# CPJKU/beat_this

Measured on NVIDIA H100. Metric: clips/sec (30 s audio->beats, final0), higher is better.
Workload: dtype f16

## Files before the change

### beat_this_b200/csrc/kernels_fused.cu

```cuda
#include <cstdio>
#include <cstdlib>
#include <cstring>

#include "tc_common.cuh"

namespace bt {

constexpr int FU_WARPS = 8;
constexpr int FU_THREADS = 32 * FU_WARPS;

__device__ __forceinline__ void stage_weight(h16* dst, const h16* __restrict__ src, int rows, int cols) {
  const int vpr = cols / 8;
  for (int i = threadIdx.x; i < rows * vpr; i += blockDim.x) {
    const int r = i / vpr, v = i - r * vpr;
    *reinterpret_cast<uint4*>(dst + r * (cols + 8) + v * 8) = __ldg(reinterpret_cast<const uint4*>(src + static_cast<int64_t>(r) * cols) + v);
  }
}
__device__ __forceinline__ uint32_t lds32(const h16* p) { return *reinterpret_cast<const uint32_t*>(p); }
template <int LD>
__device__ __forceinline__ void b_frag(const h16* sW, int nb, int ks, int lane, uint32_t& b0, uint32_t& b1) {
  const h16* p = sW + (nb * 8 + (lane >> 2)) * LD + ks * 16 + 2 * (lane & 3);
  b0 = lds32(p);
  b1 = lds32(p + 8);
}

template <int C>
__global__ void __launch_bounds__(FU_THREADS, C == 32 ? 4 : 2)
fused_qkv_kernel(const h16* __restrict__ wqkv, const float* __restrict__ X, const float* __restrict__ wg,
                 const float* __restrict__ bg, const float* __restrict__ rope_cos, const float* __restrict__ rope_sin,
                 h16* __restrict__ qkv, float* __restrict__ gates, int64_t M, int L, int F, int posmode, float qscale) {
  constexpr int LD = C + 8, KS = C / 16, NB = 3 * C / 8, heads = C / 32;
  extern __shared__ uint4 fu_smem[];
  h16* sW = reinterpret_cast<h16*>(fu_smem);
  stage_weight(sW, wqkv, 3 * C, C);
  __syncthreads();
  const int warp = threadIdx.x >> 5, lane = threadIdx.x & 31, q = lane & 3;
  const int64_t ngroups = (M + 15) / 16;
  for (int64_t g = static_cast<int64_t>(blockIdx.x) * FU_WARPS + warp; g < ngroups; g += static_cast<int64_t>(gridDim.x) * FU_WARPS) {
    int64_t m[2];
    bool ok[2];
    float xs[2][C / 4];
#pragma unroll
    for (int r = 0; r < 2; ++r) {
      m[r] = g * 16 + (lane >> 2) + 8 * r;
      ok[r] = m[r] < M;
#pragma unroll
      for (int j = 0; j < C / 4; j += 2) {
        const float2 v = ok[r] ? *reinterpret_cast<const float2*>(X + m[r] * C + 16 * (j >> 2) + 8 * ((j >> 1) & 1) + 2 * q)
                               : make_float2(0.f, 0.f);
        xs[r][j] = v.x;
        xs[r][j + 1] = v.y;
      }
    }
#pragma unroll
    for (int r = 0; r < 2; ++r) {
      float ss = 0.f;
#pragma unroll
      for (int j = 0; j < C / 4; ++j) ss = fmaf(xs[r][j], xs[r][j], ss);
      ss += __shfl_xor_sync(0xffffffffu, ss, 1);
      ss += __shfl_xor_sync(0xffffffffu, ss, 2);
      const float inv = 1.0f / fmaxf(sqrtf(ss), 1e-12f);
#pragma unroll
      for (int j = 0; j < C / 4; ++j) xs[r][j] *= inv;
    }
#pragma unroll
    for (int h = 0; h < heads; ++h) {
#pragma unroll
      for (int r = 0; r < 2; ++r) {
        float a = 0.f;
#pragma unroll
        for (int j = 0; j < C / 4; j += 2) {
          const float2 w = __ldg(reinterpret_cast<const float2*>(wg + h * C + 16 * (j >> 2) + 8 * ((j >> 1) & 1) + 2 * q));
          a = fmaf(xs[r][j], w.x, fmaf(xs[r][j + 1], w.y, a));
        }
        a += __shfl_xor_sync(0xffffffffu, a, 1);
        a += __shfl_xor_sync(0xffffffffu, a, 2);
        if (q == 0 && ok[r]) gates[m[r] * heads + h] = sigmoidf_(a + __ldg(bg + h));
      }
    }
    uint32_t a[KS][4];
#pragma unroll
    for (int ks = 0; ks < KS; ++ks) {
      a[ks][0] = pack_h16x2(xs[0][4 * ks], xs[0][4 * ks + 1]);
      a[ks][1] = pack_h16x2(xs[1][4 * ks], xs[1][4 * ks + 1]);
      a[ks][2] = pack_h16x2(xs[0][4 * ks + 2], xs[0][4 * ks + 3]);
      a[ks][3] = pack_h16x2(xs[1][4 * ks + 2], xs[1][4 * ks + 3]);
    }
    const float* cs[2];
    const float* sn[2];
#pragma unroll
    for (int r = 0; r < 2; ++r) {
      const int pos = ok[r] ? (posmode == 0 ? static_cast<int>(m[r] % L) : static_cast<int>((m[r] / L) % F)) : 0;
      cs[r] = rope_cos + pos * 16;
      sn[r] = rope_sin + pos * 16;
    }
#pragma unroll
    for (int nb = 0; nb < NB; ++nb) {
      float acc[4] = {0.f, 0.f, 0.f, 0.f};
#pragma unroll
      for (int ks = 0; ks < KS; ++ks) {
        uint32_t b0, b1;
        b_frag<LD>(sW, nb, ks, lane, b0, b1);
        mma_16816(acc, a[ks], b0, b1);
      }
      const int n = nb * 8 + 2 * q;
      const int which = (nb * 8) / C;
#pragma unroll
      for (int r = 0; r < 2; ++r) {
        float v0 = acc[2 * r], v1 = acc[2 * r + 1];
        if (which < 2) {
          const float sc = which == 0 ? qscale : 1.0f;
          const int i = ((n - which * C) & 31) >> 1;
          const float co = __ldg(cs[r] + i), si = __ldg(sn[r] + i);
          const float x0 = v0, x1 = v1;
          v0 = (x0 * co - x1 * si) * sc;
          v1 = (x1 * co + x0 * si) * sc;
        }
        if (ok[r]) *reinterpret_cast<uint32_t*>(qkv + m[r] * (3 * C) + n) = pack_h16x2(v0, v1);
      }
    }
  }
}

template <int C, bool OP>
__global__ void __launch_bounds__(FU_THREADS, C == 32 ? 3 : 2)
fused_ff_kernel(const h16* __restrict__ w1, const h16* __restrict__ w2, const h16* __restrict__ wo,
                const h16* __restrict__ O, float* __restrict__ X, const float* __restrict__ b1,
                const float* __restrict__ b2, h16* __restrict__ xb_out, int64_t M) {
  constexpr int HID = 4 * C, LD1 = C + 8, LD2 = HID + 8, KS = C / 16, NB = C / 8, HS = HID / 16;
  extern __shared__ uint4 fu_smem[];
  h16* sW1 = reinterpret_cast<h16*>(fu_smem);
  h16* sW2 = sW1 + HID * LD1;
  h16* sWo = sW2 + C * LD2;
  stage_weight(sW1, w1, HID, C);
  stage_weight(sW2, w2, C, HID);
  if constexpr (OP) stage_weight(sWo, wo, C, C);
  __syncthreads();
  const int warp = threadIdx.x >> 5, lane = threadIdx.x & 31, q = lane & 3;
  const int64_t ngroups = (M + 15) / 16;
  for (int64_t g = static_cast<int64_t>(blockIdx.x) * FU_WARPS + warp; g < ngroups; g += static_cast<int64_t>(gridDim.x) * FU_WARPS) {
    int64_t m[2];
    bool ok[2];
#pragma unroll
    for (int r = 0; r < 2; ++r) {
      m[r] = g * 16 + (lane >> 2) + 8 * r;
      ok[r] = m[r] < M;
    }
    float acc[NB][4];
#pragma unroll
    for (int nb = 0; nb < NB; ++nb)
#pragma unroll
      for (int r = 0; r < 2; ++r) {
        const float2 v = ok[r] ? *reinterpret_cast<const float2*>(X + m[r] * C + nb * 8 + 2 * q) : make_float2(0.f, 0.f);
        acc[nb][2 * r] = v.x;
        acc[nb][2 * r + 1] = v.y;
      }
    if constexpr (OP) {
      uint32_t ao[KS][4];
#pragma unroll
      for (int ks = 0; ks < KS; ++ks)
#pragma unroll
        for (int i = 0; i < 4; ++i) {
          const int r = i & 1;
          ao[ks][i] = ok[r] ? *reinterpret_cast<const uint32_t*>(O + m[r] * C + ks * 16 + 8 * (i >> 1) + 2 * q) : 0u;
        }
#pragma unroll
      for (int nb = 0; nb < NB; ++nb)
#pragma unroll
        for (int ks = 0; ks < KS; ++ks) {
          uint32_t b0, b1;
          b_frag<LD1>(sWo, nb, ks, lane, b0, b1);
          mma_16816(acc[nb], ao[ks], b0, b1);
        }
    }
    float inv[2];
#pragma unroll
    for (int r = 0; r < 2; ++r) {
      float ss = 0.f;
#pragma unroll
      for (int nb = 0; nb < NB; ++nb) ss = fmaf(acc[nb][2 * r], acc[nb][2 * r], fmaf(acc[nb][2 * r + 1], acc[nb][2 * r + 1], ss));
      ss += __shfl_xor_sync(0xffffffffu, ss, 1);
      ss += __shfl_xor_sync(0xffffffffu, ss, 2);
      inv[r] = 1.0f / fmaxf(sqrtf(ss), 1e-12f);
    }
    uint32_t a[KS][4];
#pragma unroll
    for (int ks = 0; ks < KS; ++ks) {
      a[ks][0] = pack_h16x2(acc[2 * ks][0] * inv[0], acc[2 * ks][1] * inv[0]);
      a[ks][1] = pack_h16x2(acc[2 * ks][2] * inv[1], acc[2 * ks][3] * inv[1]);
      a[ks][2] = pack_h16x2(acc[2 * ks + 1][0] * inv[0], acc[2 * ks + 1][1] * inv[0]);
      a[ks][3] = pack_h16x2(acc[2 * ks + 1][2] * inv[1], acc[2 * ks + 1][3] * inv[1]);
    }
#pragma unroll
    for (int nb = 0; nb < NB; ++nb) {
      const float2 b = __ldg(reinterpret_cast<const float2*>(b2 + nb * 8 + 2 * q));
      acc[nb][0] += b.x; acc[nb][1] += b.y;
      acc[nb][2] += b.x; acc[nb][3] += b.y;
    }
#pragma unroll 2
    for (int j = 0; j < HS; ++j) {
      float hh[2][4];
#pragma unroll
      for (int t = 0; t < 2; ++t) {
        hh[t][0] = hh[t][1] = hh[t][2] = hh[t][3] = 0.f;
#pragma unroll
        for (int ks = 0; ks < KS; ++ks) {
          uint32_t b0, b1;
          b_frag<LD1>(sW1, 2 * j + t, ks, lane, b0, b1);
          mma_16816(hh[t], a[ks], b0, b1);
        }
        const float2 b = __ldg(reinterpret_cast<const float2*>(b1 + (2 * j + t) * 8 + 2 * q));
        hh[t][0] = gelu_tanh_fast(hh[t][0] + b.x); hh[t][1] = gelu_tanh_fast(hh[t][1] + b.y);
        hh[t][2] = gelu_tanh_fast(hh[t][2] + b.x); hh[t][3] = gelu_tanh_fast(hh[t][3] + b.y);
      }
      const uint32_t ah[4] = {pack_h16x2(hh[0][0], hh[0][1]), pack_h16x2(hh[0][2], hh[0][3]), pack_h16x2(hh[1][0], hh[1][1]),
                              pack_h16x2(hh[1][2], hh[1][3])};
#pragma unroll
      for (int nb = 0; nb < NB; ++nb) {
        uint32_t b0, b1;
        b_frag<LD2>(sW2, nb, j, lane, b0, b1);
        mma_16816(acc[nb], ah, b0, b1);
      }
    }
#pragma unroll
    for (int nb = 0; nb < NB; ++nb)
#pragma unroll
      for (int r = 0; r < 2; ++r) {
        if (!ok[r]) continue;
        const int64_t o = m[r] * C + nb * 8 + 2 * q;
        *reinterpret_cast<float2*>(X + o) = make_float2(acc[nb][2 * r], acc[nb][2 * r + 1]);
        if (xb_out) *reinterpret_cast<uint32_t*>(xb_out + o) = pack_h16x2(acc[nb][2 * r], acc[nb][2 * r + 1]);
      }
  }
}

template <int C> constexpr int ff_smem(bool op) { return (4 * C * (C + 8) + C * (4 * C + 8) + (op ? C * (C + 8) : 0)) * 2; }
template <int C> constexpr int qkv_smem() { return 3 * C * (C + 8) * 2; }
template <int C> constexpr int ff_ctas() { return C == 32 ? 3 : 2; }
template <int C> constexpr int qkv_ctas() { return C == 32 ? 4 : 2; }

struct TcFfPlan {
  const void *w1, *w2, *o, *wo;
  int C;
  int64_t M;
  bool outproj;
};

TcFfPlan* tc_ff_plan_create(const void* w1_h16, const void* w2_h16, int C, int64_t M, const void* o_h16,
                            const void* wout_h16, char* err, int errlen) {
  if (C != 32 && C != 64) { snprintf(err, errlen, "fused ff: C must be 32 or 64"); return nullptr; }
  TcFfPlan* p = new TcFfPlan();
  p->w1 = w1_h16; p->w2 = w2_h16; p->o = o_h16; p->wo = wout_h16;
  p->C = C; p->M = M; p->outproj = o_h16 != nullptr && wout_h16 != nullptr;
  return p;
}
void tc_ff_plan_destroy(TcFfPlan* p) { delete p; }

static unsigned fused_grid(int64_t M, int ctas_per_sm) {
  const int64_t ctas = ((M + 15) / 16 + FU_WARPS - 1) / FU_WARPS;
  const int64_t slots = static_cast<int64_t>(g_num_sms) * ctas_per_sm;
  return static_cast<unsigned>(ctas < slots ? ctas : slots);
}

void launch_fused_ff(const TcFfPlan* p, float* X, const float* b1, const float* b2, void* xb_out, cudaStream_t st) {
  const h16* w1 = static_cast<const h16*>(p->w1);
  const h16* w2 = static_cast<const h16*>(p->w2);
  const h16* wo = static_cast<const h16*>(p->wo);
  const h16* o = static_cast<const h16*>(p->o);
  h16* xb = static_cast<h16*>(xb_out);
#define BT_FF_L(CC, OPP)                                                                                            \
  fused_ff_kernel<CC, OPP><<<fused_grid(p->M, ff_ctas<CC>()), FU_THREADS, ff_smem<CC>(OPP), st>>>(w1, w2, wo, o, X, b1, \
                                                                                                  b2, xb, p->M)
  if (p->C == 32) { if (p->outproj) BT_FF_L(32, true); else BT_FF_L(32, false); }
  else { if (p->outproj) BT_FF_L(64, true); else BT_FF_L(64, false); }
#undef BT_FF_L
}

struct TcQkvPlan {
  const void* w;
  int C;
  int64_t M;
};
TcQkvPlan* tc_qkv_plan_create(const void* wqkv_h16, int C, int64_t M, char* err, int errlen) {
  if (C != 32 && C != 64) { snprintf(err, errlen, "fused qkv: C must be 32 or 64"); return nullptr; }
  TcQkvPlan* p = new TcQkvPlan();
  p->w = wqkv_h16; p->C = C; p->M = M;
  return p;
}
void tc_qkv_plan_destroy(TcQkvPlan* p) { delete p; }
void launch_fused_qkv(const TcQkvPlan* p, const float* X, const float* wg, const float* bg, const float* rope_cos,
                      const float* rope_sin, void* qkv, float* gates, int L, int F, int posmode, float qscale,
                      cudaStream_t st) {
  const h16* w = static_cast<const h16*>(p->w);
  h16* out = static_cast<h16*>(qkv);
  if (p->C == 32)
    fused_qkv_kernel<32><<<fused_grid(p->M, qkv_ctas<32>()), FU_THREADS, qkv_smem<32>(), st>>>(w, X, wg, bg, rope_cos, rope_sin, out,
                                                                                             gates, p->M, L, F, posmode, qscale);
  else
    fused_qkv_kernel<64><<<fused_grid(p->M, qkv_ctas<64>()), FU_THREADS, qkv_smem<64>(), st>>>(w, X, wg, bg, rope_cos, rope_sin, out,
                                                                                             gates, p->M, L, F, posmode, qscale);
}

int tc_init_fused(char* err, int errlen) {
  cudaError_t r = cudaFuncSetAttribute(fused_ff_kernel<32, false>, cudaFuncAttributeMaxDynamicSharedMemorySize, ff_smem<32>(false));
  if (r == cudaSuccess) r = cudaFuncSetAttribute(fused_ff_kernel<64, false>, cudaFuncAttributeMaxDynamicSharedMemorySize, ff_smem<64>(false));
  if (r == cudaSuccess) r = cudaFuncSetAttribute(fused_ff_kernel<32, true>, cudaFuncAttributeMaxDynamicSharedMemorySize, ff_smem<32>(true));
  if (r == cudaSuccess) r = cudaFuncSetAttribute(fused_ff_kernel<64, true>, cudaFuncAttributeMaxDynamicSharedMemorySize, ff_smem<64>(true));
  if (r == cudaSuccess) r = cudaFuncSetAttribute(fused_qkv_kernel<32>, cudaFuncAttributeMaxDynamicSharedMemorySize, qkv_smem<32>());
  if (r == cudaSuccess) r = cudaFuncSetAttribute(fused_qkv_kernel<64>, cudaFuncAttributeMaxDynamicSharedMemorySize, qkv_smem<64>());
  if (r != cudaSuccess) {
    snprintf(err, errlen, "cudaFuncSetAttribute(fused_ff_kernel / fused_qkv_kernel) failed: %s", cudaGetErrorString(r));
    return -1;
  }
  return 0;
}

}
```

### beat_this_b200/csrc/kernels_misc.cu

```cuda
#include <cuda_fp16.h>
#include <cstdio>
#include <cstdlib>

#include "bt_kernels.h"
#include "common.cuh"
#include "tc_common.cuh"

namespace bt {

__global__ void __launch_bounds__(128)
stem_kernel(const float* __restrict__ spect, const ChunkSrc* __restrict__ chunks, int L,
            const float* __restrict__ bn1_scale, const float* __restrict__ bn1_shift,
            const float* __restrict__ w, const float* __restrict__ bias, float* __restrict__ out) {
  __shared__ float ws[32 * 12];
  __shared__ float bs[32];
  for (int i = threadIdx.x; i < 32 * 12; i += 128) ws[i] = w[i];
  if (threadIdx.x < 32) bs[threadIdx.x] = bias[threadIdx.x];
  __syncthreads();
  const int t = blockIdx.x * 128 + threadIdx.x;
  const int f = blockIdx.y;
  const int b = blockIdx.z;
  if (t >= L) return;
  const ChunkSrc cs = chunks[b];
  float in[4][3];
#pragma unroll
  for (int dt = 0; dt < 3; ++dt) {
    const int tl = t + dt - 1;
    const bool conv_ok = tl >= 0 && tl < cs.len;
    const int64_t fr = static_cast<int64_t>(cs.start) + tl;
    const bool clip_ok = fr >= 0 && fr < cs.T;
    float4 v = make_float4(0.f, 0.f, 0.f, 0.f);
    if (conv_ok && clip_ok)
      v = *reinterpret_cast<const float4*>(spect + (cs.frame_base + fr) * 128 + 4 * f);
    const float vv[4] = {v.x, v.y, v.z, v.w};
#pragma unroll
    for (int df = 0; df < 4; ++df)
      in[df][dt] = conv_ok ? fmaf(vv[df], bn1_scale[4 * f + df], bn1_shift[4 * f + df]) : 0.f;
  }
  float* op = out + ((static_cast<int64_t>(b) * 32 + f) * L + t) * 32;
#pragma unroll
  for (int c4 = 0; c4 < 8; ++c4) {
    float r[4];
#pragma unroll
    for (int i = 0; i < 4; ++i) {
      const int co = c4 * 4 + i;
      float a = bs[co];
#pragma unroll
      for (int df = 0; df < 4; ++df)
#pragma unroll
        for (int dt = 0; dt < 3; ++dt) a = fmaf(in[df][dt], ws[co * 12 + df * 3 + dt], a);
      r[i] = gelu_fast(a);
    }
    reinterpret_cast<float4*>(op)[c4] = make_float4(r[0], r[1], r[2], r[3]);
  }
}

__global__ void __launch_bounds__(256)
zero_tail_kernel(uint4* __restrict__ buf, const ChunkSrc* __restrict__ chunks, int F, int L, int row_vec) {
  const int plane = blockIdx.x;
  const int len = chunks[plane / F].len;
  const int64_t n = static_cast<int64_t>(L - len) * row_vec;
  uint4* p = buf + (static_cast<int64_t>(plane) * L + len) * row_vec;
  for (int64_t i = threadIdx.x; i < n; i += 256) p[i] = make_uint4(0u, 0u, 0u, 0u);
}
void launch_zero_tail(void* buf, int elem_bytes, const ChunkSrc* chunks, int nchunks, int F, int L, int C, cudaStream_t st) {
  zero_tail_kernel<<<nchunks * F, 256, 0, st>>>(reinterpret_cast<uint4*>(buf), chunks, F, L, C * elem_bytes / 16);
}

void launch_stem(const float* spect, const ChunkSrc* chunks, int nchunks, int L, const float* bn1_scale,
                 const float* bn1_shift, const float* w, const float* bias, float* out,
                 cudaStream_t st) {
  dim3 grid(ceil_div(L, 128), 32, nchunks);
  stem_kernel<<<grid, 128, 0, st>>>(spect, chunks, L, bn1_scale, bn1_shift, w, bias, out);
}

template <typename TAct, int C>
__global__ void __launch_bounds__(256)
norm_kernel(const float* __restrict__ x, TAct* __restrict__ xn, int64_t M, float* __restrict__ gates,
            const float* __restrict__ wg, const float* __restrict__ bg, int heads) {
  constexpr int LPR = C / 4 < 32 ? C / 4 : 32;
  constexpr int RPW = 32 / LPR;
  constexpr int VPL = C / 4 / LPR;
  const int lane = threadIdx.x & 31;
  const int64_t warp = static_cast<int64_t>(blockIdx.x) * 8 + (threadIdx.x >> 5);
  const int64_t row = warp * RPW + lane / LPR;
  const int li = lane % LPR;
  const bool ok = row < M;
  const float4* xr = reinterpret_cast<const float4*>(x + (ok ? row : 0) * C);
  float4 v[VPL];
  float ss = 0.f;
#pragma unroll
  for (int i = 0; i < VPL; ++i) {
    v[i] = xr[li + LPR * i];
    ss = fmaf(v[i].x, v[i].x, ss); ss = fmaf(v[i].y, v[i].y, ss);
    ss = fmaf(v[i].z, v[i].z, ss); ss = fmaf(v[i].w, v[i].w, ss);
  }
#pragma unroll
  for (int o = LPR / 2; o > 0; o >>= 1) ss += __shfl_xor_sync(0xffffffffu, ss, o);
  const float inv = 1.0f / fmaxf(sqrtf(ss), 1e-12f);
#pragma unroll
  for (int i = 0; i < VPL; ++i) { v[i].x *= inv; v[i].y *= inv; v[i].z *= inv; v[i].w *= inv; }
  if (gates) {
    for (int h = 0; h < heads; ++h) {
      const float4* w4 = reinterpret_cast<const float4*>(wg + h * C);
      float a = 0.f;
#pragma unroll
      for (int i = 0; i < VPL; ++i) {
        const float4 w = __ldg(w4 + li + LPR * i);
        a = fmaf(v[i].x, w.x, a); a = fmaf(v[i].y, w.y, a); a = fmaf(v[i].z, w.z, a); a = fmaf(v[i].w, w.w, a);
      }
#pragma unroll
      for (int o = LPR / 2; o > 0; o >>= 1) a += __shfl_xor_sync(0xffffffffu, a, o);
      if (ok && li == 0) gates[row * heads + h] = sigmoidf_(a + __ldg(bg + h));
    }
  }
  if (!ok) return;
#pragma unroll
  for (int i = 0; i < VPL; ++i) {
    TAct* dst = xn + row * C + 4 * (li + LPR * i);
    if constexpr (sizeof(TAct) == 4) {
      *reinterpret_cast<float4*>(dst) = v[i];
    } else {
      uint2 u;
      u.x = pack_h16x2(v[i].x, v[i].y);
      u.y = pack_h16x2(v[i].z, v[i].w);
      *reinterpret_cast<uint2*>(dst) = u;
    }
  }
}

template <typename TAct>
static void norm_dispatch(const float* x, void* xn, int64_t M, int C, float* gates, const float* wg, const float* bg,
                          int heads, cudaStream_t st) {
  TAct* o = reinterpret_cast<TAct*>(xn);
#define BT_NORM_CASE(c)                                                                                   \
  case c: {                                                                                               \
    constexpr int rpw = (c / 4 < 32) ? 32 / (c / 4) : 1;                                                  \
    norm_kernel<TAct, c><<<static_cast<unsigned>(ceil_div64(M, 8 * rpw)), 256, 0, st>>>(x, o, M, gates, wg, \
                                                                                          bg, heads);     \
  } break;
  switch (C) {
    BT_NORM_CASE(32) BT_NORM_CASE(64) BT_NORM_CASE(128) BT_NORM_CASE(256) BT_NORM_CASE(512) BT_NORM_CASE(1024)
    default: break;
  }
#undef BT_NORM_CASE
}

void launch_norm(const float* x, void* xn, int64_t M, int C, int act_h16, cudaStream_t st, float* gates,
                 const float* wg, const float* bg, int heads) {
  if (act_h16) norm_dispatch<h16>(x, xn, M, C, gates, wg, bg, heads, st);
  else norm_dispatch<float>(x, xn, M, C, gates, wg, bg, heads, st);
}

__device__ __forceinline__ void load_row32(const float* p, float (&v)[32]) {
#pragma unroll
  for (int i = 0; i < 8; ++i) {
    const float4 q = reinterpret_cast<const float4*>(p)[i];
    v[4 * i] = q.x; v[4 * i + 1] = q.y; v[4 * i + 2] = q.z; v[4 * i + 3] = q.w;
  }
}

template <int F>
__global__ void __launch_bounds__(128, 4)
attn_freq_kernel(const float* __restrict__ qkv, const float* __restrict__ gates, float* __restrict__ out,
                 int B, int L, int heads, float scale) {
  constexpr int GPW = 32 / F;
  constexpr int RS = 36;
  constexpr int GS = F * RS + 4;
  __shared__ __align__(16) float Ks[4][GPW * GS];
  __shared__ __align__(16) float Vs[4][GPW * GS];
  const int wib = threadIdx.x >> 5, lane = threadIdx.x & 31;
  const int g = lane / F, f = lane % F;
  const int64_t ngrp = static_cast<int64_t>(B) * L * heads;
  const int64_t grp0 = (static_cast<int64_t>(blockIdx.x) * 4 + wib) * GPW;
  if (grp0 >= ngrp) return;
  const int64_t grp = grp0 + g;
  const bool act = grp < ngrp;
  const int64_t gg = act ? grp : grp0;
  const int h = static_cast<int>(gg % heads);
  const int64_t bt_ = gg / heads;
  const int t = static_cast<int>(bt_ % L);
  const int b = static_cast<int>(bt_ / L);
  const int C = heads * 32;
  const int64_t m = (static_cast<int64_t>(b) * F + f) * L + t;
  const float* rp = qkv + m * 3 * C + h * 32;
  float q[32];
  {
    float kv[32];
    load_row32(rp + C, kv);
    float* kd = &Ks[wib][g * GS + f * RS];
#pragma unroll
    for (int i = 0; i < 8; ++i)
      reinterpret_cast<float4*>(kd)[i] = make_float4(kv[4 * i], kv[4 * i + 1], kv[4 * i + 2], kv[4 * i + 3]);
    load_row32(rp + 2 * C, kv);
    float* vd = &Vs[wib][g * GS + f * RS];
#pragma unroll
    for (int i = 0; i < 8; ++i)
      reinterpret_cast<float4*>(vd)[i] = make_float4(kv[4 * i], kv[4 * i + 1], kv[4 * i + 2], kv[4 * i + 3]);
    load_row32(rp, q);
#pragma unroll
    for (int d = 0; d < 32; ++d) q[d] *= scale;
  }
  __syncwarp();
  const float* kb = &Ks[wib][g * GS];
  const float* vb = &Vs[wib][g * GS];
  float s[F];
  float mx = -INFINITY;
#pragma unroll
  for (int j = 0; j < F; ++j) {
    float a = 0.f;
#pragma unroll
    for (int i = 0; i < 8; ++i) {
      const float4 k4 = reinterpret_cast<const float4*>(kb + j * RS)[i];
      a = fmaf(q[4 * i], k4.x, a); a = fmaf(q[4 * i + 1], k4.y, a);
      a = fmaf(q[4 * i + 2], k4.z, a); a = fmaf(q[4 * i + 3], k4.w, a);
    }
    s[j] = a;
    mx = fmaxf(mx, a);
    asm volatile("" ::: "memory");
  }
  float l = 0.f;
#pragma unroll
  for (int j = 0; j < F; ++j) {
    s[j] = __expf(s[j] - mx);
    l += s[j];
  }
  float o[32];
#pragma unroll
  for (int d = 0; d < 32; ++d) o[d] = 0.f;
#pragma unroll
  for (int j = 0; j < F; ++j) {
#pragma unroll
    for (int i = 0; i < 8; ++i) {
      const float4 v4 = reinterpret_cast<const float4*>(vb + j * RS)[i];
      o[4 * i] = fmaf(s[j], v4.x, o[4 * i]); o[4 * i + 1] = fmaf(s[j], v4.y, o[4 * i + 1]);
      o[4 * i + 2] = fmaf(s[j], v4.z, o[4 * i + 2]); o[4 * i + 3] = fmaf(s[j], v4.w, o[4 * i + 3]);
    }
    asm volatile("" ::: "memory");
  }
  if (act) {
    const float gsc = gates[m * heads + h] / l;
    float* op = out + m * C + h * 32;
#pragma unroll
    for (int i = 0; i < 8; ++i)
      reinterpret_cast<float4*>(op)[i] = make_float4(o[4 * i] * gsc, o[4 * i + 1] * gsc, o[4 * i + 2] * gsc, o[4 * i + 3] * gsc);
  }
}


constexpr int FT_TT = 4;

template <int F>
__global__ void __launch_bounds__(128)
attn_freq_mma_kernel(const __grid_constant__ CUtensorMap tmIn, const __grid_constant__ CUtensorMap tmOut,
                     const float* __restrict__ gates, int L, int heads, float scale_log2) {
  constexpr int GPW = 32 / F;
  constexpr int NT = F == 32 ? 4 : 2;
  constexpr int HEADS = 4 * GPW / FT_TT;
  constexpr int C = HEADS * 32;
  constexpr int PH_BYTES = F * FT_TT * 64;
  extern __shared__ uint8_t smem_raw[];
  const uint32_t sbase = (smem_u32(smem_raw) + 1023u) & ~1023u;
  const uint32_t sIn = sbase;
  const uint32_t sOut = sIn + 3 * HEADS * PH_BYTES;
  const uint32_t bar = sOut + F * FT_TT * C * 2;
  const int wib = threadIdx.x >> 5, lane = threadIdx.x & 31;
  const int t0 = blockIdx.x * FT_TT, b = blockIdx.y;
  if (threadIdx.x == 0) {
    mbar_init(bar, 1);
    fence_barrier_init();
    mbar_expect_tx(bar, 3 * HEADS * PH_BYTES);
    for (int part = 0; part < 3; ++part)
      for (int h = 0; h < HEADS; ++h)
        tma_load_3d(sIn + (part * HEADS + h) * PH_BYTES, &tmIn, bar, part * C + h * 32, b * F, t0);
  }
  __syncthreads();
  mbar_wait(bar, 0);
  const int h = (wib * GPW) / FT_TT;
  const int tt_base = (wib * GPW) % FT_TT;
  auto row_addr = [&](uint32_t base, int r, int chunk) -> uint32_t {
    const int row = tt_base * F + r;
    return base + row * 64 + ((chunk ^ ((row >> 1) & 3)) << 4);
  };
  const uint32_t sQ = sIn + (0 * HEADS + h) * PH_BYTES, sK = sIn + (1 * HEADS + h) * PH_BYTES, sV = sIn + (2 * HEADS + h) * PH_BYTES;
  const int g = lane >> 2, c = lane & 3;
#pragma unroll
  for (int mt = 0; mt < 2; ++mt) {
    const int key_base = F == 32 ? 0 : 16 * mt;
    uint32_t qa[2][4];
#pragma unroll
    for (int kk = 0; kk < 2; ++kk)
      ldmatrix_x4(row_addr(sQ, 16 * mt + (lane & 7) + ((lane >> 3) & 1) * 8, kk * 2 + (lane >> 4)), qa[kk]);
    float sc[NT][4];
#pragma unroll
    for (int j = 0; j < NT; ++j) {
      sc[j][0] = sc[j][1] = sc[j][2] = sc[j][3] = 0.f;
      uint32_t kb[4];
      ldmatrix_x4(row_addr(sK, key_base + 8 * j + (lane & 7), lane >> 3), kb);
      mma_16816(sc[j], qa[0], kb[0], kb[1]);
      mma_16816(sc[j], qa[1], kb[2], kb[3]);
    }
    if (F == 8) {
      sc[1][0] = sc[1][1] = -INFINITY;
      sc[0][2] = sc[0][3] = -INFINITY;
    }
    float mx0 = -INFINITY, mx1 = -INFINITY;
#pragma unroll
    for (int j = 0; j < NT; ++j) {
      mx0 = fmaxf(mx0, fmaxf(sc[j][0], sc[j][1]));
      mx1 = fmaxf(mx1, fmaxf(sc[j][2], sc[j][3]));
    }
    mx0 = fmaxf(mx0, __shfl_xor_sync(0xffffffffu, mx0, 1)); mx0 = fmaxf(mx0, __shfl_xor_sync(0xffffffffu, mx0, 2));
    mx1 = fmaxf(mx1, __shfl_xor_sync(0xffffffffu, mx1, 1)); mx1 = fmaxf(mx1, __shfl_xor_sync(0xffffffffu, mx1, 2));
    float l0 = 0.f, l1 = 0.f;
#pragma unroll
    for (int j = 0; j < NT; ++j) {
      sc[j][0] = exp2f((sc[j][0] - mx0) * scale_log2); sc[j][1] = exp2f((sc[j][1] - mx0) * scale_log2);
      sc[j][2] = exp2f((sc[j][2] - mx1) * scale_log2); sc[j][3] = exp2f((sc[j][3] - mx1) * scale_log2);
      l0 += sc[j][0] + sc[j][1];
      l1 += sc[j][2] + sc[j][3];
    }
    l0 += __shfl_xor_sync(0xffffffffu, l0, 1); l0 += __shfl_xor_sync(0xffffffffu, l0, 2);
    l1 += __shfl_xor_sync(0xffffffffu, l1, 1); l1 += __shfl_xor_sync(0xffffffffu, l1, 2);
    float o[4][4];
#pragma unroll
    for (int jd = 0; jd < 4; ++jd) o[jd][0] = o[jd][1] = o[jd][2] = o[jd][3] = 0.f;
#pragma unroll
    for (int kk = 0; kk < NT / 2; ++kk) {
      uint32_t pa[4];
      pa[0] = pack_h16x2(sc[2 * kk][0], sc[2 * kk][1]);
      pa[1] = pack_h16x2(sc[2 * kk][2], sc[2 * kk][3]);
      pa[2] = pack_h16x2(sc[2 * kk + 1][0], sc[2 * kk + 1][1]);
      pa[3] = pack_h16x2(sc[2 * kk + 1][2], sc[2 * kk + 1][3]);
#pragma unroll
      for (int jd = 0; jd < 4; jd += 2) {
        uint32_t vb[4];
        const int q4 = lane >> 3;
        ldmatrix_x4_trans(row_addr(sV, key_base + 16 * kk + (q4 & 1) * 8 + (lane & 7), jd + (q4 >> 1)), vb);
        mma_16816(o[jd], pa, vb[0], vb[1]);
        mma_16816(o[jd + 1], pa, vb[2], vb[3]);
      }
    }
#pragma unroll
    for (int half = 0; half < 2; ++half) {
      const int r = 16 * mt + g + 8 * half;
      const int f = r % F, tt = tt_base + r / F;
      const int t = t0 + tt;
      const int64_t m = (static_cast<int64_t>(b) * F + f) * L + (t < L ? t : L - 1);
      const float gsc = gates[m * HEADS + h] / (half == 0 ? l0 : l1);
      const uint32_t orow = sOut + (tt * F + f) * (C * 2) + h * 64;
#pragma unroll
      for (int jd = 0; jd < 4; ++jd)
        asm volatile("st.shared.b32 [%0], %1;" ::"r"(orow + (4 * jd + c) * 4), "r"(pack_h16x2(o[jd][2 * half] * gsc, o[jd][2 * half + 1] * gsc)) : "memory");
    }
  }
  fence_proxy_async_smem();
  __syncthreads();
  if (threadIdx.x == 0) {
    tma_store_3d(&tmOut, sOut, 0, b * F, t0);
    bulk_commit();
    bulk_wait_read<0>();
  }
}

#define BT_FREQ_TC_INSTANCES(X) X(32) X(16) X(8)
template <int F> constexpr int freq_tc_heads() { return 4 * (32 / F) / FT_TT; }
template <int F> constexpr int freq_tc_smem() {
  return 3 * freq_tc_heads<F>() * F * FT_TT * 64 + F * FT_TT * freq_tc_heads<F>() * 32 * 2 + 1024 + 64;
}

struct TcFreqPlan {
  CUtensorMap tmIn;
  CUtensorMap tmOut;
  int B, F, L;
};

TcFreqPlan* tc_freq_plan_create(const void* qkv, void* out, int B, int F, int L, int heads, char* err, int errlen) {
  bool ok = false;
#define BT_FREQ_OK(FF) ok = ok || (F == FF && heads == freq_tc_heads<FF>());
  BT_FREQ_TC_INSTANCES(BT_FREQ_OK)
#undef BT_FREQ_OK
  if (!ok) {
    snprintf(err, errlen, "frequency attention: no tensor-core kernel for F = %d with %d heads (F = 32, 16, 8 take 1, 2, 4 "
             "heads)", F, heads);
    return nullptr;
  }
  TcFreqPlan* p = new TcFreqPlan();
  p->B = B; p->F = F; p->L = L;
  const int C = heads * 32;
  const uint64_t din[3] = {static_cast<uint64_t>(3 * C), static_cast<uint64_t>(B) * F, static_cast<uint64_t>(L)};
  const uint64_t sin_[2] = {static_cast<uint64_t>(L) * 3 * C * 2, static_cast<uint64_t>(3 * C) * 2};
  const uint32_t bin[3] = {32, static_cast<uint32_t>(F), FT_TT};
  const uint64_t dout[3] = {static_cast<uint64_t>(C), static_cast<uint64_t>(B) * F, static_cast<uint64_t>(L)};
  const uint64_t sout[2] = {static_cast<uint64_t>(L) * C * 2, static_cast<uint64_t>(C) * 2};
  const uint32_t bout[3] = {static_cast<uint32_t>(C), static_cast<uint32_t>(F), FT_TT};
  if (!make_tmap(&p->tmIn, qkv, 3, din, sin_, bin, 64, err, errlen) || !make_tmap(&p->tmOut, out, 3, dout, sout, bout, 0, err, errlen)) {
    delete p;
    return nullptr;
  }
  return p;
}
void tc_freq_plan_destroy(TcFreqPlan* p) { delete p; }

void launch_attn_freq_tc(const TcFreqPlan* p, const float* gates, float scale, cudaStream_t st) {
  const float sl2 = scale * 1.4426950408889634f;
  const dim3 grid(ceil_div(p->L, FT_TT), p->B);
#define BT_FREQ_LAUNCH(FF)                                                                                             \
  if (p->F == FF)                                                                                                      \
    attn_freq_mma_kernel<FF><<<grid, 128, freq_tc_smem<FF>(), st>>>(p->tmIn, p->tmOut, gates, p->L, freq_tc_heads<FF>(), sl2);
  BT_FREQ_TC_INSTANCES(BT_FREQ_LAUNCH)
#undef BT_FREQ_LAUNCH
}

int tc_init_attn_freq(char* err, int errlen) {
  cudaError_t r = cudaSuccess;
#define BT_FREQ_ATTR(FF) \
  if (r == cudaSuccess) r = cudaFuncSetAttribute(attn_freq_mma_kernel<FF>, cudaFuncAttributeMaxDynamicSharedMemorySize, freq_tc_smem<FF>());
  BT_FREQ_TC_INSTANCES(BT_FREQ_ATTR)
#undef BT_FREQ_ATTR
  if (r != cudaSuccess) {
    snprintf(err, errlen, "cudaFuncSetAttribute(attn_freq_mma_kernel) failed: %s", cudaGetErrorString(r));
    return -1;
  }
  return 0;
}

void launch_attn_freq_simt(const float* qkv, const float* gates, float* out, int B, int F, int L, int heads, float scale,
                           cudaStream_t st) {
  const int64_t ngrp = static_cast<int64_t>(B) * L * heads;
  const unsigned grid = static_cast<unsigned>(ceil_div64(ngrp, 4 * (32 / F)));
  if (F == 32) attn_freq_kernel<32><<<grid, 128, 0, st>>>(qkv, gates, out, B, L, heads, scale);
  else if (F == 16) attn_freq_kernel<16><<<grid, 128, 0, st>>>(qkv, gates, out, B, L, heads, scale);
  else attn_freq_kernel<8><<<grid, 128, 0, st>>>(qkv, gates, out, B, L, heads, scale);
}

__global__ void __launch_bounds__(256)
head_kernel(const float* __restrict__ x, int D, const float* __restrict__ w, const float* __restrict__ bias,
            const ChunkSrc* __restrict__ chunks, int nchunks, int L, float* __restrict__ beat,
            float* __restrict__ down, int sum_head) {
  const int64_t row = static_cast<int64_t>(blockIdx.x) * 8 + (threadIdx.x >> 5);
  const int lane = threadIdx.x & 31;
  if (row >= static_cast<int64_t>(nchunks) * L) return;
  const int b = static_cast<int>(row / L), t = static_cast<int>(row % L);
  const ChunkSrc cs = chunks[b];
  if (t < cs.write_lo || t >= cs.write_hi) return;
  const float* xr = x + row * D;
  float ss = 0.f, a0 = 0.f, a1 = 0.f;
  for (int i = lane; i < D; i += 32) {
    const float v = xr[i];
    ss = fmaf(v, v, ss);
    a0 = fmaf(v, __ldg(w + i), a0);
    a1 = fmaf(v, __ldg(w + D + i), a1);
  }
  ss = warp_sum(ss); a0 = warp_sum(a0); a1 = warp_sum(a1);
  if (lane == 0) {
    const float inv = 1.0f / fmaxf(sqrtf(ss), 1e-12f);
    const float o0 = a0 * inv + bias[0], o1 = a1 * inv + bias[1];
    const int64_t fr = cs.out_base + cs.start + t;
    beat[fr] = sum_head ? o0 + o1 : o0;
    down[fr] = o1;
  }
}

void launch_head(const float* x, int D, const float* w, const float* b, const ChunkSrc* chunks,
                 int nchunks, int L, float* beat, float* down, int sum_head, cudaStream_t st) {
  const int64_t rows = static_cast<int64_t>(nchunks) * L;
  head_kernel<<<static_cast<unsigned>(ceil_div64(rows, 8)), 256, 0, st>>>(x, D, w, b, chunks, nchunks, L,
                                                                           beat, down, sum_head);
}

__device__ int compact_peaks(const float* __restrict__ x, int T, double* __restrict__ frames, int cap,
                             int* s_warp, int* s_base) {
  const int tid = threadIdx.x, lane = tid & 31, wid = tid >> 5;
  if (tid == 0) *s_base = 0;
  __syncthreads();
  for (int t0 = 0; t0 < T; t0 += 256) {
    const int t = t0 + tid;
    bool pk = false;
    if (t < T) {
      const float v = x[t];
      float mx = v;
#pragma unroll
      for (int d = -3; d <= 3; ++d) {
        const int u = t + d;
        if (u >= 0 && u < T) mx = fmaxf(mx, x[u]);
      }
      pk = (v == mx) && (v > 0.f);
    }
    const unsigned bal = __ballot_sync(0xffffffffu, pk);
    if (lane == 0) s_warp[wid] = __popc(bal);
    __syncthreads();
    int off = *s_base;
    for (int w = 0; w < wid; ++w) off += s_warp[w];
    if (pk) {
      const int idx = off + __popc(bal & ((1u << lane) - 1));
      if (idx < cap) frames[idx] = static_cast<double>(t);
    }
    __syncthreads();
    if (tid == 0) {
      int tot = 0;
      for (int w = 0; w < 8; ++w) tot += s_warp[w];
      *s_base += tot;
    }
    __syncthreads();
  }
  return *s_base;
}

__device__ int dedup_to_times(double* p, int n, double fps) {
  if (n == 0) return 0;
  int out = 0;
  double cur = p[0];
  double c = 1.0;
  for (int i = 1; i < n; ++i) {
    const double p2 = p[i];
    if (p2 - cur <= 1.0) {
      c += 1.0;
      cur += (p2 - cur) / c;
    } else {
      p[out++] = cur / fps;
      cur = p2;
      c = 1.0;
    }
  }
  p[out++] = cur / fps;
  return out;
}

__global__ void __launch_bounds__(256)
peakpick_kernel(const float* __restrict__ beat, const float* __restrict__ down,
                const int64_t* __restrict__ frame_off, double* __restrict__ beat_t, int32_t* __restrict__ n_beat,
                double* __restrict__ down_t, int32_t* __restrict__ n_down, int max_peaks, double fps) {
  __shared__ int s_warp[8];
  __shared__ int s_base;
  const int clip = blockIdx.x;
  const int64_t f0 = frame_off[clip];
  const int T = static_cast<int>(frame_off[clip + 1] - f0);
  double* bt_ = beat_t + static_cast<int64_t>(clip) * max_peaks;
  double* dt_ = down_t + static_cast<int64_t>(clip) * max_peaks;
  const int nb_raw = compact_peaks(beat + f0, T, bt_, max_peaks, s_warp, &s_base);
  __syncthreads();
  const int nd_raw = compact_peaks(down + f0, T, dt_, max_peaks, s_warp, &s_base);
  __syncthreads();
  __shared__ int s_nb, s_nd;
  if (threadIdx.x == 0) {
    if (nb_raw > max_peaks || nd_raw > max_peaks) {
      n_beat[clip] = nb_raw;
      n_down[clip] = nd_raw;
      s_nb = -1;
    } else {
      s_nb = dedup_to_times(bt_, nb_raw, fps);
      s_nd = dedup_to_times(dt_, nd_raw, fps);
    }
  }
  __syncthreads();
  const int nb = s_nb;
  if (nb < 0) return;
  int nd = s_nd;
  if (nb > 0) {
    for (int i = threadIdx.x; i < nd; i += blockDim.x) {
      const double d = dt_[i];
      int best = 0;
      double bd = fabs(bt_[0] - d);
      for (int j = 1; j < nb; ++j) {
        const double dd = fabs(bt_[j] - d);
        if (dd < bd) { bd = dd; best = j; }
      }
      dt_[i] = bt_[best];
    }
  }
  __syncthreads();
  if (threadIdx.x == 0) {
    for (int i = 1; i < nd; ++i) {
      const double v = dt_[i];
      int j = i - 1;
      while (j >= 0 && dt_[j] > v) { dt_[j + 1] = dt_[j]; --j; }
      dt_[j + 1] = v;
    }
    int o = 0;
    for (int i = 0; i < nd; ++i)
      if (o == 0 || dt_[i] != dt_[o - 1]) dt_[o++] = dt_[i];
    nd = o;
    n_beat[clip] = nb;
    n_down[clip] = nd;
  }
}

void launch_peakpick(const float* beat, const float* down, const int64_t* frame_off_dev, int n_clips,
                     double* beat_t, int32_t* n_beat, double* down_t, int32_t* n_down, int max_peaks,
                     double fps, cudaStream_t st) {
  if (n_clips <= 0) return;
  peakpick_kernel<<<n_clips, 256, 0, st>>>(beat, down, frame_off_dev, beat_t, n_beat, down_t, n_down,
                                           max_peaks, fps);
}

__global__ void f32_to_h16_kernel(const float* __restrict__ in, h16* __restrict__ out, int64_t n) {
  const int64_t i = static_cast<int64_t>(blockIdx.x) * blockDim.x + threadIdx.x;
  if (i < n) out[i] = to_out<h16>(in[i]);
}
__global__ void h16_to_f32_kernel(const h16* __restrict__ in, float* __restrict__ out, int64_t n) {
  const int64_t i = static_cast<int64_t>(blockIdx.x) * blockDim.x + threadIdx.x;
  if (i < n) out[i] = to_f32(in[i]);
}
void launch_f32_to_h16(const float* in, void* out, int64_t n, cudaStream_t st) {
  if (n <= 0) return;
  f32_to_h16_kernel<<<static_cast<unsigned>(ceil_div64(n, 256)), 256, 0, st>>>(in, reinterpret_cast<h16*>(out), n);
}
void launch_h16_to_f32(const void* in, float* out, int64_t n, cudaStream_t st) {
  if (n <= 0) return;
  h16_to_f32_kernel<<<static_cast<unsigned>(ceil_div64(n, 256)), 256, 0, st>>>(reinterpret_cast<const h16*>(in), out, n);
}

template <typename TAct>
__global__ void pack_qkv_test_kernel(const float* __restrict__ q, const float* __restrict__ k,
                                     const float* __restrict__ v, TAct* __restrict__ qkv, int seqs, int L,
                                     int heads, float qscale) {
  const int C = heads * 32;
  const int64_t i = static_cast<int64_t>(blockIdx.x) * blockDim.x + threadIdx.x;
  const int64_t n = static_cast<int64_t>(seqs) * L * C;
  if (i >= n) return;
  const int c = static_cast<int>(i % C);
  const int64_t m = i / C;
  qkv[m * 3 * C + c] = to_out<TAct>(q[i] * qscale);
  qkv[m * 3 * C + C + c] = to_out<TAct>(k[i]);
  qkv[m * 3 * C + 2 * C + c] = to_out<TAct>(v[i]);
}
void launch_pack_qkv_test(const float* q, const float* k, const float* v, void* qkv, int seqs, int L, int heads,
                          float qscale, int act_h16, cudaStream_t st) {
  const int64_t n = static_cast<int64_t>(seqs) * L * heads * 32;
  const unsigned grid = static_cast<unsigned>(ceil_div64(n, 256));
  if (act_h16)
    pack_qkv_test_kernel<h16><<<grid, 256, 0, st>>>(q, k, v, reinterpret_cast<h16*>(qkv), seqs, L, heads, qscale);
  else
    pack_qkv_test_kernel<float><<<grid, 256, 0, st>>>(q, k, v, reinterpret_cast<float*>(qkv), seqs, L, heads, qscale);
}

}
```

Before: 786.3.

## Stage fused-kernel activations via cp.async, use ldmatrix B fragments, widen stores

```diff
diff --git a/beat_this_b200/csrc/kernels_fused.cu b/beat_this_b200/csrc/kernels_fused.cu
--- a/beat_this_b200/csrc/kernels_fused.cu
+++ b/beat_this_b200/csrc/kernels_fused.cu
@@ -16,12 +16,45 @@
     *reinterpret_cast<uint4*>(dst + r * (cols + 8) + v * 8) = __ldg(reinterpret_cast<const uint4*>(src + static_cast<int64_t>(r) * cols) + v);
   }
 }
-__device__ __forceinline__ uint32_t lds32(const h16* p) { return *reinterpret_cast<const uint32_t*>(p); }
 template <int LD>
-__device__ __forceinline__ void b_frag(const h16* sW, int nb, int ks, int lane, uint32_t& b0, uint32_t& b1) {
-  const h16* p = sW + (nb * 8 + (lane >> 2)) * LD + ks * 16 + 2 * (lane & 3);
-  b0 = lds32(p);
-  b1 = lds32(p + 8);
+__device__ __forceinline__ void b_frag_k2(uint32_t sW, int nb, int ks, int lane, uint32_t (&b)[4]) {
+  ldmatrix_x4(sW + 2 * ((nb * 8 + (lane & 7)) * LD + ks * 16 + 8 * (lane >> 3)), b);
+}
+template <int LD>
+__device__ __forceinline__ void b_frag_n2(uint32_t sW, int nb, int ks, int lane, uint32_t (&b)[4]) {
+  ldmatrix_x4(sW + 2 * ((nb * 8 + (lane & 7) + 8 * (lane >> 4)) * LD + ks * 16 + 8 * ((lane >> 3) & 1)), b);
+}
+
+__device__ __forceinline__ int quad_col(int q) { return 8 * (q & 1) + 2 * (q & 2); }
+__device__ __forceinline__ uint2 quad_pair(uint32_t lo, uint32_t hi, int q) {
+  const uint32_t other = __shfl_xor_sync(0xffffffffu, (q & 1) ? lo : hi, 1);
+  return (q & 1) ? make_uint2(other, hi) : make_uint2(lo, other);
+}
+
+template <int C> __host__ __device__ constexpr int stage_floats() { return 16 * C + 96; }
+template <int C>
+__device__ __forceinline__ int stage_idx(int r, int col) { return r * C + 8 * (r & 3) + 24 * (r >> 2) + col; }
+__device__ __forceinline__ void cp_async16(uint32_t dst, const void* src, bool ok) {
+  asm volatile("cp.async.cg.shared.global [%0], [%1], 16, %2;" ::"r"(dst), "l"(src), "r"(ok ? 16 : 0) : "memory");
+}
+__device__ __forceinline__ void cp_async_commit() { asm volatile("cp.async.commit_group;" ::: "memory"); }
+__device__ __forceinline__ void cp_async_wait_all() { asm volatile("cp.async.wait_group 0;" ::: "memory"); }
+template <int C>
+__device__ __forceinline__ void stage_rows(uint32_t st, const float* __restrict__ X, int64_t g, int64_t ngroups,
+                                           int64_t M, int lane) {
+  constexpr int CPR = C / 4;
+  if (g < ngroups) {
+#pragma unroll
+    for (int t = 0; t < 16 * CPR / 32; ++t) {
+      const int r = (lane >> 3) + 4 * (t / (CPR / 8)), k = (lane & 7) + 8 * (t % (CPR / 8));
+      cp_async16(st + 4 * stage_idx<C>(r, 4 * k), X + (g * 16 + r) * C + 4 * k, g * 16 + r < M);
+    }
+  }
+  cp_async_commit();
+}
+template <int C>
+__device__ __forceinline__ float2 stage_f2(uint32_t st, int r, int col) {
+  return ld_shared_v2_f32(st + 4 * stage_idx<C>(r, col));
 }
 
 template <int C>
@@ -29,25 +62,29 @@
 fused_qkv_kernel(const h16* __restrict__ wqkv, const float* __restrict__ X, const float* __restrict__ wg,
                  const float* __restrict__ bg, const float* __restrict__ rope_cos, const float* __restrict__ rope_sin,
                  h16* __restrict__ qkv, float* __restrict__ gates, int64_t M, int L, int F, int posmode, float qscale) {
-  constexpr int LD = C + 8, KS = C / 16, NB = 3 * C / 8, heads = C / 32;
+  constexpr int LD = C + 8, KS = C / 16, heads = C / 32;
   extern __shared__ uint4 fu_smem[];
   h16* sW = reinterpret_cast<h16*>(fu_smem);
+  const int warp = threadIdx.x >> 5, lane = threadIdx.x & 31, q = lane & 3;
+  const uint32_t sw = smem_u32(sW), st = sw + 2 * 3 * C * LD + 4 * warp * stage_floats<C>();
+  const int64_t ngroups = (M + 15) / 16;
+  int64_t g = static_cast<int64_t>(blockIdx.x) * FU_WARPS + warp;
+  stage_rows<C>(st, X, g, ngroups, M, lane);
   stage_weight(sW, wqkv, 3 * C, C);
   __syncthreads();
-  const int warp = threadIdx.x >> 5, lane = threadIdx.x & 31, q = lane & 3;
-  const int64_t ngroups = (M + 15) / 16;
-  for (int64_t g = static_cast<int64_t>(blockIdx.x) * FU_WARPS + warp; g < ngroups; g += static_cast<int64_t>(gridDim.x) * FU_WARPS) {
+  for (; g < ngroups; g += static_cast<int64_t>(gridDim.x) * FU_WARPS) {
     int64_t m[2];
     bool ok[2];
     float xs[2][C / 4];
+    cp_async_wait_all();
+    __syncwarp();
 #pragma unroll
     for (int r = 0; r < 2; ++r) {
       m[r] = g * 16 + (lane >> 2) + 8 * r;
       ok[r] = m[r] < M;
 #pragma unroll
       for (int j = 0; j < C / 4; j += 2) {
-        const float2 v = ok[r] ? *reinterpret_cast<const float2*>(X + m[r] * C + 16 * (j >> 2) + 8 * ((j >> 1) & 1) + 2 * q)
-                               : make_float2(0.f, 0.f);
+        const float2 v = stage_f2<C>(st, (lane >> 2) + 8 * r, 16 * (j >> 2) + 8 * ((j >> 1) & 1) + 2 * q);
         xs[r][j] = v.x;
         xs[r][j + 1] = v.y;
       }
@@ -86,6 +123,8 @@
       a[ks][2] = pack_h16x2(xs[0][4 * ks + 2], xs[0][4 * ks + 3]);
       a[ks][3] = pack_h16x2(xs[1][4 * ks + 2], xs[1][4 * ks + 3]);
     }
+    __syncwarp();
+    stage_rows<C>(st, X, g + static_cast<int64_t>(gridDim.x) * FU_WARPS, ngroups, M, lane);
     const float* cs[2];
     const float* sn[2];
 #pragma unroll
@@ -94,29 +133,39 @@
       cs[r] = rope_cos + pos * 16;
       sn[r] = rope_sin + pos * 16;
     }
-#pragma unroll
-    for (int nb = 0; nb < NB; ++nb) {
-      float acc[4] = {0.f, 0.f, 0.f, 0.f};
-#pragma unroll
-      for (int ks = 0; ks < KS; ++ks) {
-        uint32_t b0, b1;
-        b_frag<LD>(sW, nb, ks, lane, b0, b1);
-        mma_16816(acc, a[ks], b0, b1);
-      }
-      const int n = nb * 8 + 2 * q;
-      const int which = (nb * 8) / C;
+#pragma unroll 1
+    for (int which = 0; which < 3; ++which)
+#pragma unroll
+    for (int nb = which * (C / 8); nb < (which + 1) * (C / 8); nb += 2) {
+      float acc[2][4] = {};
+#pragma unroll
+      for (int u = 0; u < 2; ++u)
+#pragma unroll
+        for (int ks = 0; ks < KS; ks += 2) {
+          uint32_t b[4];
+          b_frag_k2<LD>(sw, nb + u, ks, lane, b);
+          mma_16816(acc[u], a[ks], b[0], b[1]);
+          mma_16816(acc[u], a[ks + 1], b[2], b[3]);
+        }
 #pragma unroll
       for (int r = 0; r < 2; ++r) {
-        float v0 = acc[2 * r], v1 = acc[2 * r + 1];
-        if (which < 2) {
-          const float sc = which == 0 ? qscale : 1.0f;
-          const int i = ((n - which * C) & 31) >> 1;
-          const float co = __ldg(cs[r] + i), si = __ldg(sn[r] + i);
-          const float x0 = v0, x1 = v1;
-          v0 = (x0 * co - x1 * si) * sc;
-          v1 = (x1 * co + x0 * si) * sc;
-        }
-        if (ok[r]) *reinterpret_cast<uint32_t*>(qkv + m[r] * (3 * C) + n) = pack_h16x2(v0, v1);
+        uint32_t p[2];
+#pragma unroll
+        for (int u = 0; u < 2; ++u) {
+          const int n = (nb + u) * 8 + 2 * q;
+          float v0 = acc[u][2 * r], v1 = acc[u][2 * r + 1];
+          if (which < 2) {
+            const float sc = which == 0 ? qscale : 1.0f;
+            const int i = ((n - which * C) & 31) >> 1;
+            const float co = __ldg(cs[r] + i), si = __ldg(sn[r] + i);
+            const float x0 = v0, x1 = v1;
+            v0 = (x0 * co - x1 * si) * sc;
+            v1 = (x1 * co + x0 * si) * sc;
+          }
+          p[u] = pack_h16x2(v0, v1);
+        }
+        const uint2 w = quad_pair(p[0], p[1], q);
+        if (ok[r]) *reinterpret_cast<uint2*>(qkv + m[r] * (3 * C) + nb * 8 + quad_col(q)) = w;
       }
     }
   }
@@ -132,13 +181,25 @@
   h16* sW1 = reinterpret_cast<h16*>(fu_smem);
   h16* sW2 = sW1 + HID * LD1;
   h16* sWo = sW2 + C * LD2;
+  const int warp = threadIdx.x >> 5, lane = threadIdx.x & 31, q = lane & 3;
+  const uint32_t sw1 = smem_u32(sW1), sw2 = smem_u32(sW2), swo = smem_u32(sWo);
+  const uint32_t st = swo + 2 * (OP ? C * LD1 : 0) + 4 * warp * stage_floats<C>();
+  const int64_t ngroups = (M + 15) / 16;
+  int64_t g = static_cast<int64_t>(blockIdx.x) * FU_WARPS + warp;
+  auto prefetch_o = [&](int64_t gg) {
+    if (OP && lane == 0 && gg < ngroups) {
+      const int64_t rows = M - gg * 16 < 16 ? M - gg * 16 : 16;
+      asm volatile("cp.async.bulk.prefetch.L2.global [%0], %1;" ::"l"(O + gg * 16 * C), "r"(static_cast<uint32_t>(rows * C * 2))
+                   : "memory");
+    }
+  };
+  stage_rows<C>(st, X, g, ngroups, M, lane);
+  prefetch_o(g);
   stage_weight(sW1, w1, HID, C);
   stage_weight(sW2, w2, C, HID);
   if constexpr (OP) stage_weight(sWo, wo, C, C);
   __syncthreads();
-  const int warp = threadIdx.x >> 5, lane = threadIdx.x & 31, q = lane & 3;
-  const int64_t ngroups = (M + 15) / 16;
-  for (int64_t g = static_cast<int64_t>(blockIdx.x) * FU_WARPS + warp; g < ngroups; g += static_cast<int64_t>(gridDim.x) * FU_WARPS) {
+  for (; g < ngroups; g += static_cast<int64_t>(gridDim.x) * FU_WARPS) {
     int64_t m[2];
     bool ok[2];
 #pragma unroll
@@ -147,14 +208,19 @@
       ok[r] = m[r] < M;
     }
     float acc[NB][4];
+    cp_async_wait_all();
+    __syncwarp();
 #pragma unroll
     for (int nb = 0; nb < NB; ++nb)
 #pragma unroll
       for (int r = 0; r < 2; ++r) {
-        const float2 v = ok[r] ? *reinterpret_cast<const float2*>(X + m[r] * C + nb * 8 + 2 * q) : make_float2(0.f, 0.f);
+        const float2 v = stage_f2<C>(st, (lane >> 2) + 8 * r, nb * 8 + 2 * q);
         acc[nb][2 * r] = v.x;
         acc[nb][2 * r + 1] = v.y;
       }
+    __syncwarp();
+    stage_rows<C>(st, X, g + static_cast<int64_t>(gridDim.x) * FU_WARPS, ngroups, M, lane);
+    prefetch_o(g + static_cast<int64_t>(gridDim.x) * FU_WARPS);
     if constexpr (OP) {
       uint32_t ao[KS][4];
 #pragma unroll
@@ -167,10 +233,11 @@
 #pragma unroll
       for (int nb = 0; nb < NB; ++nb)
 #pragma unroll
-        for (int ks = 0; ks < KS; ++ks) {
-          uint32_t b0, b1;
-          b_frag<LD1>(sWo, nb, ks, lane, b0, b1);
-          mma_16816(acc[nb], ao[ks], b0, b1);
+        for (int ks = 0; ks < KS; ks += 2) {
+          uint32_t b[4];
+          b_frag_k2<LD1>(swo, nb, ks, lane, b);
+          mma_16816(acc[nb], ao[ks], b[0], b[1]);
+          mma_16816(acc[nb], ao[ks + 1], b[2], b[3]);
         }
     }
     float inv[2];
@@ -204,10 +271,11 @@
       for (int t = 0; t < 2; ++t) {
         hh[t][0] = hh[t][1] = hh[t][2] = hh[t][3] = 0.f;
 #pragma unroll
-        for (int ks = 0; ks < KS; ++ks) {
-          uint32_t b0, b1;
-          b_frag<LD1>(sW1, 2 * j + t, ks, lane, b0, b1);
-          mma_16816(hh[t], a[ks], b0, b1);
+        for (int ks = 0; ks < KS; ks += 2) {
+          uint32_t b[4];
+          b_frag_k2<LD1>(sw1, 2 * j + t, ks, lane, b);
+          mma_16816(hh[t], a[ks], b[0], b[1]);
+          mma_16816(hh[t], a[ks + 1], b[2], b[3]);
         }
         const float2 b = __ldg(reinterpret_cast<const float2*>(b1 + (2 * j + t) * 8 + 2 * q));
         hh[t][0] = gelu_tanh_fast(hh[t][0] + b.x); hh[t][1] = gelu_tanh_fast(hh[t][1] + b.y);
@@ -216,10 +284,11 @@
       const uint32_t ah[4] = {pack_h16x2(hh[0][0], hh[0][1]), pack_h16x2(hh[0][2], hh[0][3]), pack_h16x2(hh[1][0], hh[1][1]),
                               pack_h16x2(hh[1][2], hh[1][3])};
 #pragma unroll
-      for (int nb = 0; nb < NB; ++nb) {
-        uint32_t b0, b1;
-        b_frag<LD2>(sW2, nb, j, lane, b0, b1);
-        mma_16816(acc[nb], ah, b0, b1);
+      for (int nb = 0; nb < NB; nb += 2) {
+        uint32_t b[4];
+        b_frag_n2<LD2>(sw2, nb, j, lane, b);
+        mma_16816(acc[nb], ah, b[0], b[1]);
+        mma_16816(acc[nb + 1], ah, b[2], b[3]);
       }
     }
 #pragma unroll
@@ -234,8 +303,10 @@
   }
 }
 
-template <int C> constexpr int ff_smem(bool op) { return (4 * C * (C + 8) + C * (4 * C + 8) + (op ? C * (C + 8) : 0)) * 2; }
-template <int C> constexpr int qkv_smem() { return 3 * C * (C + 8) * 2; }
+template <int C> constexpr int ff_smem(bool op) {
+  return (4 * C * (C + 8) + C * (4 * C + 8) + (op ? C * (C + 8) : 0)) * 2 + FU_WARPS * stage_floats<C>() * 4;
+}
+template <int C> constexpr int qkv_smem() { return 3 * C * (C + 8) * 2 + FU_WARPS * stage_floats<C>() * 4; }
 template <int C> constexpr int ff_ctas() { return C == 32 ? 3 : 2; }
 template <int C> constexpr int qkv_ctas() { return C == 32 ? 4 : 2; }
 
@@ -301,13 +372,21 @@
                                                                                              gates, p->M, L, F, posmode, qscale);
 }
 
+template <typename K>
+static cudaError_t fused_attrs(K* kernel, int smem, bool max_carveout = false) {
+  cudaError_t r = cudaFuncSetAttribute(kernel, cudaFuncAttributeMaxDynamicSharedMemorySize, smem);
+  if (r == cudaSuccess && max_carveout)
+    r = cudaFuncSetAttribute(kernel, cudaFuncAttributePreferredSharedMemoryCarveout, cudaSharedmemCarveoutMaxShared);
+  return r;
+}
+
 int tc_init_fused(char* err, int errlen) {
-  cudaError_t r = cudaFuncSetAttribute(fused_ff_kernel<32, false>, cudaFuncAttributeMaxDynamicSharedMemorySize, ff_smem<32>(false));
-  if (r == cudaSuccess) r = cudaFuncSetAttribute(fused_ff_kernel<64, false>, cudaFuncAttributeMaxDynamicSharedMemorySize, ff_smem<64>(false));
-  if (r == cudaSuccess) r = cudaFuncSetAttribute(fused_ff_kernel<32, true>, cudaFuncAttributeMaxDynamicSharedMemorySize, ff_smem<32>(true));
-  if (r == cudaSuccess) r = cudaFuncSetAttribute(fused_ff_kernel<64, true>, cudaFuncAttributeMaxDynamicSharedMemorySize, ff_smem<64>(true));
-  if (r == cudaSuccess) r = cudaFuncSetAttribute(fused_qkv_kernel<32>, cudaFuncAttributeMaxDynamicSharedMemorySize, qkv_smem<32>());
-  if (r == cudaSuccess) r = cudaFuncSetAttribute(fused_qkv_kernel<64>, cudaFuncAttributeMaxDynamicSharedMemorySize, qkv_smem<64>());
+  cudaError_t r = fused_attrs(fused_ff_kernel<32, false>, ff_smem<32>(false));
+  if (r == cudaSuccess) r = fused_attrs(fused_ff_kernel<64, false>, ff_smem<64>(false), true);
+  if (r == cudaSuccess) r = fused_attrs(fused_ff_kernel<32, true>, ff_smem<32>(true));
+  if (r == cudaSuccess) r = fused_attrs(fused_ff_kernel<64, true>, ff_smem<64>(true), true);
+  if (r == cudaSuccess) r = fused_attrs(fused_qkv_kernel<32>, qkv_smem<32>());
+  if (r == cudaSuccess) r = fused_attrs(fused_qkv_kernel<64>, qkv_smem<64>());
   if (r != cudaSuccess) {
     snprintf(err, errlen, "cudaFuncSetAttribute(fused_ff_kernel / fused_qkv_kernel) failed: %s", cudaGetErrorString(r));
     return -1;
diff --git a/beat_this_b200/csrc/kernels_misc.cu b/beat_this_b200/csrc/kernels_misc.cu
--- a/beat_this_b200/csrc/kernels_misc.cu
+++ b/beat_this_b200/csrc/kernels_misc.cu
@@ -20,7 +20,6 @@
   const int t = blockIdx.x * 128 + threadIdx.x;
   const int f = blockIdx.y;
   const int b = blockIdx.z;
-  if (t >= L) return;
   const ChunkSrc cs = chunks[b];
   float in[4][3];
 #pragma unroll
@@ -37,13 +36,14 @@
     for (int df = 0; df < 4; ++df)
       in[df][dt] = conv_ok ? fmaf(vv[df], bn1_scale[4 * f + df], bn1_shift[4 * f + df]) : 0.f;
   }
-  float* op = out + ((static_cast<int64_t>(b) * 32 + f) * L + t) * 32;
-#pragma unroll
-  for (int c4 = 0; c4 < 8; ++c4) {
-    float r[4];
-#pragma unroll
-    for (int i = 0; i < 4; ++i) {
-      const int co = c4 * 4 + i;
+  const bool odd = t & 1;
+  float* op = out + ((static_cast<int64_t>(b) * 32 + f) * L + (t & ~1)) * 32 + (odd ? 4 : 0);
+#pragma unroll
+  for (int c8 = 0; c8 < 4; ++c8) {
+    float r[8];
+#pragma unroll
+    for (int i = 0; i < 8; ++i) {
+      const int co = c8 * 8 + i;
       float a = bs[co];
 #pragma unroll
       for (int df = 0; df < 4; ++df)
@@ -51,7 +51,13 @@
         for (int dt = 0; dt < 3; ++dt) a = fmaf(in[df][dt], ws[co * 12 + df * 3 + dt], a);
       r[i] = gelu_fast(a);
     }
-    reinterpret_cast<float4*>(op)[c4] = make_float4(r[0], r[1], r[2], r[3]);
+    float x[4];
+#pragma unroll
+    for (int i = 0; i < 4; ++i) x[i] = __shfl_xor_sync(0xffffffffu, odd ? r[i] : r[4 + i], 1);
+    const float4 lo = odd ? make_float4(x[0], x[1], x[2], x[3]) : make_float4(r[0], r[1], r[2], r[3]);
+    const float4 hi = odd ? make_float4(r[4], r[5], r[6], r[7]) : make_float4(x[0], x[1], x[2], x[3]);
+    if ((t & ~1) < L) reinterpret_cast<float4*>(op + 8 * c8)[0] = lo;
+    if ((t | 1) < L) reinterpret_cast<float4*>(op + 32 + 8 * c8)[0] = hi;
   }
 }
 
```

Result: faster. 813.4, median of 6 (+3.4%).
